# microsoft/ISLE

Measured on AMD Instinct MI355X. Metric: docs/sec end-to-end ISLETrain (SVD+k-means), k=1000; top-k σ rel-err, higher is better.
Workload: dtype f32

## Files before the change

isle_amd/csrc/api.cpp:

```cpp
#include <algorithm>
#include <chrono>
#include <cmath>
#include <cstdarg>
#include <cstdlib>
#include <cstring>
#include <numeric>
#include <thread>

#include <dlfcn.h>

#include "api_internal.h"

int isle_fail(isle_ctx* c, int code, const char* fmt, ...) {
  char buf[1024];
  va_list ap;
  va_start(ap, fmt);
  vsnprintf(buf, sizeof buf, fmt, ap);
  va_end(ap);
  if (c) c->err = buf;
  return code;
}

const IsleKnobInfo isle_knob_table[KN_COUNT] = {
    {"ISLE_GRAM_LDS", "form", "0: Gram apply and k-wide products by the row-gather kernels (any CSC matrix) instead of the LDS-banded form (row-constant B)"},
// ... 6 lines not shown
    {"ISLE_GL_PANEL", "tuning", "8 | 10: columns per pass of the k-wide / thin products (default 10, 8 at 8 items per lane in pass 1)"},
    {"ISLE_GL_WIDE_GROUPED", "tuning", "0: every panel pass of the projection writes its 40 bytes straight into the documents' rows of P (default on a large shard: the panels' rows go whole and in position order into a scratch, sixteen at a time, and a second kernel assembles 640-byte pieces of the document-major rows and the rows' squared norms)"},
    {"ISLE_WIDE_GATHER", "form", "k-wide products (projection, first word-space assignment) by the row-gather kernel"},
    {"ISLE_WIDE_LDS", "form", "k-wide products through the LDS-banded pass-1 stream whatever the vocabulary size"},
    {"ISLE_KS_ROWSHARD", "form", "0: every rank orthogonalises the whole Krylov block (default with several ranks: row slices, all-reduced coefficients, all-gathered block)"},
    {"ISLE_KS_SYNC", "form", "expand loop without the speculative pipeline (one host synchronisation per step)"},
    {"ISLE_KS_ORTHO_PASSES", "form", "3: the reference's three Gram-Schmidt passes per Krylov step instead of two"},
    {"ISLE_UPDATE_MFMA", "form", "0: the orthogonalisation's update F -= V H by FMA chains with the coefficients read from LDS (update_k) instead of on the matrix cores (same sums in another order)"},
    {"ISLE_EVD_JACOBI", "form", "small symmetric EVD by block Jacobi instead of tridiagonalisation"},
    {"ISLE_TD_CHAIN", "form", "tridiagonalisation as a launch chain instead of the persistent kernel"},
    {"ISLE_TD_BAR", "tuning", "flat | hier: the persistent tridiagonalisation crosses its grid barriers on one counter (gb_barrier) or through the hierarchical barrier (gbh_barrier) instead of the sharded counters polled together (gbs_barrier, gridbar.h; round 6: 36.4 / 37.0 / 40.7 ms per EVD at n = 2000 sharded / hier / flat); same bits"},
    {"ISLE_TD_BACK", "form", "seq: the eigenvectors' back-transformation applies the reflectors one by one (td_back_k) instead of by blocks of four in compact WY form"},
    {"ISLE_EVD_SPLIT", "form", "1: with several ranks rank r computes the eigenvectors [r kc, (r + 1) kc) of the small EVD and the columns are all-gathered (same bits on every rank; default since round 6: every rank computes all of them — the stage's kernels are chains of n steps whatever the number of vectors, the split saves no time)"},
    {"ISLE_KMPP_HOST_DICE", "form", "k-means++ dice scaled and searched through the host round trip (the multi-rank form) on one rank too"},
    {"ISLE_KMPP_SPARSE", "form", "0 / 1: k-means++ rounds on the projection / through thin products of B (default: by cost)"},
    {"ISLE_KMPP_TRACK", "form", "0: Lloyd in span(U) always starts with a full assignment pass (default at k > 224 on a large shard: it starts from the nearest seeds and tile minima the k-means++ rounds kept)"},
    {"ISLE_NO_HAMERLY", "form", "both Lloyd loops without distance bounds (every document re-examined every iteration)"},
    {"ISLE_KMEANS_BOUNDS", "form", "hamerly | none: bounds of Lloyd on B (default Yinyang group bounds)"},
    {"ISLE_PROJ_BOUNDS", "form", "hamerly: single lower bound in the projected Lloyd loop at k > 224 instead of tile bounds"},
    {"ISLE_PROJ_FULL", "form", "gemm | fused: full passes of the projected Lloyd loop as GEMM + epilogue or as the fused register kernel"},
    {"ISLE_FIRST_ASSIGN", "form", "sparse | projection: first assignment of Lloyd on B through the sparse product or through the projection"},
    {"ISLE_GEMM_BF16X3", "form", "0: the D x k x k dot products of the assignment steps on the f32 matrix cores (gemm_f32.h) instead of the bf16 ones with operands split in three terms (gemm_bf16x3.h)"},
    {"ISLE_GEMM_EPILOGUE", "form", "0: the D x k x k products of the assignment steps are written to memory and read by dots_assign_cm_k / proj_dots_tiles_k instead of the epilogues inside the product (same bits)"},
    {"ISLE_GEMM_TERMS", "form", "3: the assignment products run once with three bf16 terms per operand (default: two terms first, the rows whose arg-min that leaves open again with three; same assignment)"},
    {"ISLE_GEMM_DMA", "form", "0: the two-term pass of the assignment products splits A on the fly and stages it through registers (gemm_bf16x3_k) instead of reading the projection's pre-split copy by LDS-DMA through a ring of stages (gemm_bf16x2_dma_k; same products in the same order: same bits)"},
    {"ISLE_YY_MODE", "form", "doc | docg | group: Yinyang iteration by document (row-major / group-major centres) or ordered by group (default: group at k >= 256)"},
    {"ISLE_YY_FUSED", "form", "0: the by-group Yinyang iteration lowers the bounds (yy_filter_k) and tightens the active documents (yy2_tighten_k) in two launches instead of one (same bits)"},
    {"ISLE_YY_MOVERS", "form", "0: every centre's movement lowers its Yinyang group's bound (default: up to ten centres that moved far beyond the rest are bounded by their exact new distances instead)"},
    {"ISLE_YY_REGROUP", "form", "0: a Yinyang group is eight consecutive centres (default at k >= 256 behind the product's first assignment: the centres in the order of their squared norms, so that the few centres every far-off document is near share groups; same partitions, a third of the (document, group) pairs)"},
    {"ISLE_YY_ORDER", "form", "doc | member: the Yinyang filter visits the documents in their own order or in the member lists' (default: doc for the fused by-group launch, member otherwise; same bits)"},
// ... 635 lines not shown
```

isle_amd/csrc/common.h:

```cpp
#pragma once
#include <hip/hip_runtime.h>
#include <rccl/rccl.h>

#include <atomic>
#include <cstdint>
#include <cstdio>
#include <functional>
#include <string>
#include <thread>
#include <vector>

struct IsleLaunchRefused {
  const char* file = nullptr;
  int line = 0;
  unsigned long long threads = 0;
};
inline IsleLaunchRefused& isle_launch_refused() {
  static thread_local IsleLaunchRefused r;
  return r;
}
inline bool isle_launch_fits(dim3 g, dim3 b, const char* file, int line) {
  const unsigned long long blocks = (unsigned long long)g.x * g.y * g.z, threads = blocks * ((unsigned long long)b.x * b.y * b.z);
  if (threads < (1ull << 32)) return true;
  IsleLaunchRefused& r = isle_launch_refused();
// ... 56 lines not shown
    hipError_t e = hipHostMalloc((void**)&p, n, hipHostMallocDefault);
    if (e == hipSuccess) cap = n;
    return e;
  }
  PinBuf() = default;
  PinBuf(const PinBuf&) = delete;
  PinBuf& operator=(const PinBuf&) = delete;
  ~PinBuf() {
    if (p) (void)hipHostFree(p);
  }
};

enum IsleKnob {
  KN_GRAM_LDS, KN_GL_G1, KN_GL_G2, KN_GL_PLACE, KN_GL_FILL_BUCKETS, KN_GL_ROUNDS, KN_GL_COLUMNS, KN_GL_PANEL, KN_GL_WIDE_GROUPED, KN_WIDE_GATHER, KN_WIDE_LDS,
  KN_KS_ROWSHARD, KN_KS_SYNC, KN_KS_ORTHO_PASSES, KN_UPDATE_MFMA, KN_EVD_JACOBI, KN_TD_CHAIN, KN_TD_BAR, KN_TD_BACK, KN_EVD_SPLIT,
  KN_KMPP_HOST_DICE, KN_KMPP_SPARSE, KN_KMPP_TRACK, KN_NO_HAMERLY, KN_KMEANS_BOUNDS, KN_PROJ_BOUNDS, KN_PROJ_FULL, KN_FIRST_ASSIGN, KN_GEMM_BF16X3, KN_GEMM_EPILOGUE, KN_GEMM_TERMS, KN_GEMM_DMA, KN_YY_MODE, KN_YY_FUSED, KN_YY_MOVERS, KN_YY_REGROUP, KN_YY_ORDER, KN_PT_SORT, KN_PROJ_ACTIVE, KN_PROJ_SUMS, KN_CENTERS_FRESH,
  KN_INFER_CAP_ROWS, KN_CHUNK_COLS, KN_COMM_TIMEOUT, KN_COMM_SELFTEST, KN_FORCE_COMM, KN_TEST_STALL_MS,
  KN_ROCTX, KN_HOST_TRACE, KN_DEBUG_HAMERLY, KN_DEBUG_EVD, KN_GL_VERBOSE, KN_TD_FORCE_BAIL_RANK, KN_GL_TEST_CUS, KN_GL_ABLATE_SKIP,
  KN_COUNT
};
struct IsleKnobInfo {
  const char* name;
  const char* kind;
  const char* what;
};
extern const IsleKnobInfo isle_knob_table[KN_COUNT];

struct GlDesc {
  uint32_t wave0, wstride, nw, b0, b1, slab, pos_base, pad;
};
struct GlSide {
  uint32_t n_out = 0, n_src = 0, NB = 0, nslice = 0, nwv = 0, ndesc = 0;
  int G = 4;
  uint32_t wpg = 16;
  DevBuf<uint32_t> slice_of;
  DevBuf<int64_t> roff;
  DevBuf<uint16_t> cnt;
  DevBuf<uint2> ids;
  DevBuf<GlDesc> desc;
  int64_t total_sr = 0;
};

struct IslePinSmall {
  double kmpp_stage[(128u << 10) / 8];
// ... 215 lines not shown
  DevBuf<float> ptlb;
  DevBuf<uint32_t> pneed;
  DevBuf<uint32_t> pcand;
  DevBuf<int> seg_desc;
  DevBuf<float> seg_part;
  DevBuf<uint32_t> proj_counted;
  DevBuf<uint32_t> proj_nch;
  DevBuf<float> proj_dpart;
  DevBuf<float> Csum_local;
  DevBuf<uint32_t> active;
  DevBuf<unsigned long long> dbg_cnt;
  DevBuf<uint32_t> kmpp_arg;
  DevBuf<float> kmpp_m2a;
  DevBuf<float> kmpp_tmin;
  DevBuf<float> kmpp_best;
  bool kmpp_track = false;
  int kmpp_track_seeds = 0;
  int kmpp_track_k = 0;
  uint64_t P_gen = 0, kmpp_P_gen = 0;
  std::vector<float> kmpp_C_host;
  DevBuf<float> yy_cg;
  DevBuf<uint32_t> yy_map;
  DevBuf<float> yy_cns;
  DevBuf<float> yy_liftC;
  DevBuf<uint32_t> yy_own, yy_res;
  DevBuf<unsigned long long> yy_need;
  DevBuf<uint32_t> yy_cnt, yy_off;
  DevBuf<uint8_t> yy_pgrp;
  DevBuf<float> centers_old;
  DevBuf<float> Pa, pna, Cold;
// ... 119 lines not shown
int k_ham_delta(isle_ctx* c, float* delta_dev , int k, HamTop* top_dev);
int k_hamerly_filter(isle_ctx* c, const uint32_t* order, const uint32_t* assign, float* ub, float* lb, const float* delta_dev, const HamTop* top_dev,
                     uint32_t* active, uint32_t* nactive, int fam = ISLE_T_SPARSE_ASSIGN);
int k_csc_validate(isle_ctx* c, unsigned long long* err_host2);
int k_doc_norms(isle_ctx* c, float* dn);
int k_centers_from_rows(isle_ctx* c, const uint32_t* assign, int k, int ldk, float* Crm, bool first_of_run = true);
int k_pt_filter(isle_ctx* c, const uint32_t* order, const uint32_t* assign, float* ub, float* tlb, int T, int TL, const float* delta_dev,
                const float* tmove_dev, uint32_t* need, uint32_t* active, uint32_t* nactive, const YyMovers& mv, const float* mdots, const float* cn, const float* pn);
int k_pt_tighten(isle_ctx* c, const float* P, const float* pn, int ldk, const float* C, const float* cn, const uint32_t* assign, const uint32_t* cand,
                 const uint32_t* ncand, float* ub, const float* tlb, int T, int TL, uint32_t* need, uint32_t* active, uint32_t* nactive);
int k_gl_detect(isle_ctx* c);
int k_centers_counts(isle_ctx* c, const uint32_t* assign, int k, int ldk, float* Crm, bool fresh);
int k_gl_build(isle_ctx* c);
int k_gl_wide(isle_ctx* c, const float* Mrm, int k, int ld, float* Out, float* norms = nullptr ,
              void* A2pos = nullptr , bool* a2_done = nullptr);
int k_gl_thin(isle_ctx* c, const float* Wcm, int nc, int ld, float* Out, bool by_position = false);
int k_gl_apply_cm(isle_ctx* c, const float* Xcm, int b, int BP, float* Zcm);
int k_gl_panel_width(const isle_ctx* c);

int k_th_stats(isle_ctx* c, uint64_t* tokens_nz_dev);
int k_th_round_hist(isle_ctx* c, float avg, uint32_t maxv);
int k_th_zetas(isle_ctx* c, uint32_t maxv, uint64_t count_gr, uint64_t count_eq);
int k_th_count(isle_ctx* c, bool with_weights);
int k_th_drop(isle_ctx* c, const uint8_t* drop_dev);
int k_th_scans(isle_ctx* c);
int k_th_emit(isle_ctx* c, uint64_t doc_base);

int k_sort_pairs_u64(isle_ctx* c, uint64_t* key_a, uint32_t* val_a, uint64_t* key_b, uint32_t* val_b, uint64_t n, int key_bits, bool* in_a);
int k_ingest_tdf(isle_ctx* c, const unsigned char* text_dev, uint64_t n, uint64_t V, uint64_t D, uint64_t* entries_read, uint64_t* err_out);
int k_feed_chunk(isle_ctx* c, const uint32_t* docs, const uint32_t* words, const uint32_t* counts, uint64_t n, uint64_t* bad);
int k_feed_finalize(isle_ctx* c);
// ... 108 lines not shown
```

isle_amd/csrc/gram_lds.hip:

```cpp
#include <algorithm>
#include <cstdio>
#include <cstdlib>
#include <vector>

#include "common.h"
#include "scan.h"

namespace {

constexpr int GL_WAVES = 16;
constexpr int GL_THREADS = GL_WAVES * 64;
constexpr int GL_GMAX = 8;
#ifndef GL_RB_V
#define GL_RB_V 4078
#endif
#ifndef GL_APPLY_WAVES_V
#define GL_APPLY_WAVES_V 16
#endif
constexpr uint32_t GL_RB = GL_RB_V;
constexpr uint32_t GL_APPLY_WAVES = GL_APPLY_WAVES_V;
constexpr uint32_t GL_NZ = 16;
constexpr uint32_t GL_PS = GL_RB + GL_NZ;
constexpr uint32_t GL_PSB = GL_PS * 16;
__host__ __device__ constexpr uint32_t gl_img_bytes(int LPE, bool half) { return GL_RB * (16u * (uint32_t)(half ? LPE - 1 : LPE) + (half ? 8u : 0u)); }
// ... 671 lines not shown
#define gl_ld_ids(p) gl_ld_ids_nt(p)
#else
#define gl_ld_ids(p) (*(p))
#endif

#ifndef GL_STAMPS
#define GL_STAMPS 0
#endif
#if GL_STAMPS
__device__ unsigned long long gl_stamp_acc[8];
#define GL_STAMP(var) const unsigned long long var = __builtin_amdgcn_s_memtime()
#else
#define GL_STAMP(var)
#endif

template <int LPE, bool HALF, int G>
__global__ __launch_bounds__(GL_THREADS) void gl_apply_k(const float4* __restrict__ In, uint32_t n_src, const uint2* __restrict__ ids,
                                                          const int64_t* __restrict__ roff, const uint16_t* __restrict__ cnt,
                                                          const uint32_t* __restrict__ slice_of, const GlDesc* __restrict__ desc, uint32_t NB,
                                                          float4* __restrict__ Out, size_t slab_stride, uint32_t n_out,
                                                          const uint32_t* __restrict__ rowmap ,
                                                          uint32_t out_ld4 ,
                                                          uint32_t out_n2 ) {
  extern __shared__ float4 xs[];
  constexpr int NF = HALF ? LPE - 1 : LPE;
  constexpr int NFA = NF > 0 ? NF : 1;
  constexpr uint32_t IMG = gl_img_bytes(LPE, HALF);
  constexpr int NPIECE = NF * 64 + (HALF ? 32 : 0);
  constexpr int GL_INFLIGHT = G * (4 * NF + (HALF ? 2 : 0)) <= 56 ? 4 : 2;
  const GlDesc ds = desc[blockIdx.x];
  const int lane = threadIdx.x & 63;
  const int w = __builtin_amdgcn_readfirstlane((int)(threadIdx.x >> 6));
  const int nwaves = (int)(blockDim.x >> 6);
  const bool wvalid = (uint32_t)w < ds.nw;
  const size_t wv = wvalid ? (size_t)ds.wave0 + (size_t)w * ds.wstride : (size_t)ds.wave0;
  constexpr uint32_t P0 = HALF ? GL_PS * 8u : 0u;
  uint32_t p0s = P0;
  asm volatile("" : "+s"(p0s));
// ... 108 lines not shown
    atomicAdd(&gl_stamp_acc[2], st_b2);
    atomicAdd(&gl_stamp_acc[3], st_walk);
    atomicAdd(&gl_stamp_acc[4], st_sr);
    atomicAdd(&gl_stamp_acc[5], 1ull);
    atomicAdd(&gl_stamp_acc[6], (unsigned long long)(ds.b1 - ds.b0));
  }
#endif
  if (!wvalid) return;
  if ((GL_ABLATE & 64) && (q2.x ^ q3.y) == 0x12345u) acc[0][0].x += 1.f;
  float4* out = Out + (size_t)ds.slab * slab_stride;
#pragma unroll
  for (int g = 0; g < G; ++g) {
    const uint32_t sl = slice_of[wv * G + g];
    const uint64_t pos = (uint64_t)sl * 64 + lane;
    if (sl != GL_NONE && pos < n_out) {
      if (out_n2 == GL_OUT_PLANAR) {
        const uint32_t ob = (uint32_t)pos / GL_RB, orow = (uint32_t)pos - ob * GL_RB;
        char* o = reinterpret_cast<char*>(Out) + (size_t)ob * IMG;
#pragma unroll
        for (int l = 0; l < NF; ++l) *reinterpret_cast<float4*>(o + (size_t)l * GL_RB * 16u + (size_t)orow * 16u) = acc[g][l];
        if (HALF) *reinterpret_cast<float2*>(o + (size_t)NF * GL_RB * 16u + (size_t)orow * 8u) = acch[g];
        continue;
      }
      const size_t row = rowmap ? (size_t)rowmap[pos] : (size_t)(pos - ds.pos_base);
      if (out_n2) {
        float2* o2 = reinterpret_cast<float2*>(out) + row * (size_t)out_ld4 * 2;
#pragma unroll
        for (int l = 0; l < NF; ++l) {
          if (2u * l < out_n2) o2[2 * l] = make_float2(acc[g][l].x, acc[g][l].y);
          if (2u * l + 1 < out_n2) o2[2 * l + 1] = make_float2(acc[g][l].z, acc[g][l].w);
// ... 254 lines not shown
    const bool place = !c->knob_zero(KN_GL_PLACE);
    for (size_t sid0 = 0; sid0 < nsl; sid0 += (size_t)8 << 22) {
      const dim3 grid((unsigned)cdiv((long)std::min<size_t>(nsl - sid0, (size_t)8 << 22), 8));
      if (place) {
        hipLaunchKernelGGL((gl_place_k<4, 0>), grid, dim3(512), 0, c->stream, s.NB, s.G, sid0, nsl, s.cnt.p, s.roff.p, s.ids.p);
        hipLaunchKernelGGL((gl_place_k<GL_PLACE_MAXN, 4>), grid, dim3(512), 0, c->stream, s.NB, s.G, sid0, nsl, s.cnt.p, s.roff.p, s.ids.p);
      }
      hipLaunchKernelGGL(gl_scale_ids_k, grid, dim3(512), 0, c->stream, s.G, sid0, nsl, place ? (uint32_t)GL_PLACE_MAXN : 0u, s.cnt.p, s.roff.p, s.ids.p);
      HIPCHK(c, hipGetLastError());
    }
  }
  HIPCHK(c, hipMemsetD16Async((hipDeviceptr_t)(ids16 + n16_body), (unsigned short)(GL_RB * 8), n16_all - n16_body, c->stream));
  return 0;
}

template <int LPE, bool HALF, int G>
int launch_apply_g(isle_ctx* c, const GlSide& s, const float4* In, float4* Out, size_t slab_stride, const uint32_t* rowmap, uint32_t out_ld4,
                   uint32_t out_n2) {
  constexpr uint32_t lds = (uint32_t)(HALF ? LPE - 1 : LPE) * GL_PSB + (HALF ? GL_PS * 8u : 0u);
  ISLECHK(isle_max_lds(c, (const void*)gl_apply_k<LPE, HALF, G>, (int)lds));
  hipLaunchKernelGGL((gl_apply_k<LPE, HALF, G>), dim3(s.ndesc), dim3(64 * s.wpg), lds, c->stream, In, s.n_src, s.ids.p, s.roff.p, s.cnt.p,
                     s.slice_of.p, s.desc.p, s.NB, Out, slab_stride, s.n_out, rowmap, out_ld4 ? out_ld4 : (uint32_t)LPE, out_n2);
  HIPCHK(c, hipGetLastError());
  return 0;
}
template <int LPE, bool HALF>
int launch_apply(isle_ctx* c, const GlSide& s, const float4* In, float4* Out, size_t slab_stride, const uint32_t* rowmap = nullptr,
                 uint32_t out_ld4 = 0, uint32_t out_n2 = 0) {
  switch (s.G) {
    case 4: return launch_apply_g<LPE, HALF, 4>(c, s, In, Out, slab_stride, rowmap, out_ld4, out_n2);
    case 5: return launch_apply_g<LPE, HALF, 5>(c, s, In, Out, slab_stride, rowmap, out_ld4, out_n2);
    case 6: return launch_apply_g<LPE, HALF, 6>(c, s, In, Out, slab_stride, rowmap, out_ld4, out_n2);
    case 7: return launch_apply_g<LPE, HALF, 7>(c, s, In, Out, slab_stride, rowmap, out_ld4, out_n2);
    case 8: return launch_apply_g<LPE, HALF, 8>(c, s, In, Out, slab_stride, rowmap, out_ld4, out_n2);
  }
  return isle_fail(c, ISLE_E_ARG, "LDS Gram apply: %d items per lane", s.G);
}
int launch_apply_any(isle_ctx* c, int LPE, bool half, const GlSide& s, const float4* In, float4* Out, size_t slab_stride, uint32_t out_n2) {
  if (LPE == 1) return half ? launch_apply<1, true>(c, s, In, Out, slab_stride, nullptr, 0, out_n2) : launch_apply<1, false>(c, s, In, Out, slab_stride, nullptr, 0, out_n2);
  if (LPE == 2) return half ? launch_apply<2, true>(c, s, In, Out, slab_stride, nullptr, 0, out_n2) : launch_apply<2, false>(c, s, In, Out, slab_stride, nullptr, 0, out_n2);
  if (LPE == 3 && half) return launch_apply<3, true>(c, s, In, Out, slab_stride, nullptr, 0, out_n2);
  return isle_fail(c, ISLE_E_ARG, "LDS Gram apply: a panel of %d columns", 4 * LPE);
}
// ... 401 lines not shown
  HIPCHK(c, hipGetLastError());
  return 0;
}

static int gl_panel_width(const isle_ctx* c) {
  const char* e = c->knob(KN_GL_PANEL);
  if (e && atoi(e) == 10) return 10;
  if (e && atoi(e) == 8) return 8;
  return c->gl1.G <= 7 ? 10 : 8;
}

static inline int gl_panel_store_cols(int j0, int ncol, int k, int ld) { return j0 + ncol >= k ? ld - j0 : ncol; }
static inline int gl_panel_cols(int PW, int j0, int k, int ld) { return k - j0 <= PW && ld - j0 > 10 ? 8 : std::min(PW, k - j0); }

static int gl_panel_pass(isle_ctx* c, int wcols, int j0, int ld, float* Out, float* scratch = nullptr ,
                         bool by_position = false ) {
  const int LPE = (wcols + 3) / 4;
  const bool half = wcols <= 4 * LPE - 2;
  const float4* in = (const float4*)c->gl_Xs.p;
  if (scratch) {
    float4* so = (float4*)scratch;
    if (LPE == 1) return half ? launch_apply<1, true>(c, c->gl1, in, so, 0, nullptr, 3, 0) : launch_apply<1, false>(c, c->gl1, in, so, 0, nullptr, 3, 0);
    if (LPE == 2) return half ? launch_apply<2, true>(c, c->gl1, in, so, 0, nullptr, 3, 0) : launch_apply<2, false>(c, c->gl1, in, so, 0, nullptr, 3, 0);
    if (LPE == 3 && half) return launch_apply<3, true>(c, c->gl1, in, so, 0, nullptr, 3, 0);
    return isle_fail(c, ISLE_E_ARG, "LDS products: a panel of %d stored columns", wcols);
  }
  const uint32_t ld4 = (uint32_t)(ld / 4);
  float4* out = (float4*)(Out + j0);
  const uint32_t n2 = (j0 % 4) || half ? (uint32_t)((wcols + 1) / 2) : 0u;
  const uint32_t* rowmap = by_position ? nullptr : c->dperm.p;
  if (LPE == 1) return half ? launch_apply<1, true>(c, c->gl1, in, out, 0, rowmap, ld4, n2) : launch_apply<1, false>(c, c->gl1, in, out, 0, rowmap, ld4, n2);
  if (LPE == 2) return half ? launch_apply<2, true>(c, c->gl1, in, out, 0, rowmap, ld4, n2) : launch_apply<2, false>(c, c->gl1, in, out, 0, rowmap, ld4, n2);
  if (LPE == 3 && half) return launch_apply<3, true>(c, c->gl1, in, out, 0, rowmap, ld4, n2);
  return isle_fail(c, ISLE_E_ARG, "LDS products: a panel of %d stored columns", wcols);
}

int k_gl_panel_width(const isle_ctx* c) { return gl_panel_width(c); }

int k_gl_thin(isle_ctx* c, const float* Wcm, int nc, int ld, float* Out, bool by_position) {
  ISLECHK(k_band_build(c));
  if (c->gl_mode != 1) return isle_fail(c, ISLE_E_ARG, "k_gl_thin needs the LDS-banded form");
  if (ld % 4 || nc > ld) return isle_fail(c, ISLE_E_ARG, "k_gl_thin: bad leading dimension");
  const uint32_t V = (uint32_t)c->V;
  HIPCHK(c, c->gl_Xs.reserve(gl_packed_floats(V, 3, true)));
  const int PW = gl_panel_width(c);
  for (int j0 = 0, ncol; j0 < nc; j0 += ncol) {
    ncol = gl_panel_cols(PW, j0, nc, ld);
    const int wcols = gl_panel_store_cols(j0, ncol, nc, ld);
    const int LPE = (wcols + 3) / 4;
    const bool half = wcols <= 4 * LPE - 2;
    const size_t n4 = (size_t)V * LPE;
    hipLaunchKernelGGL(gl_pack_scale_k, dim3(cdiv((long)n4, 256)), dim3(256), 0, c->stream, Wcm + (size_t)j0 * V, (size_t)V, ncol, LPE, (int)half,
                       c->rowval.p, (char*)c->gl_Xs.p);
    HIPCHK(c, hipGetLastError());
    ISLECHK(gl_panel_pass(c, wcols, j0, ld, Out, nullptr, by_position));
  }
  return 0;
}

constexpr int GL_WG_PANELS = 16;
struct GlWidePanels {
  int n;
  int j0[GL_WG_PANELS];
  int w[GL_WG_PANELS];
  int ncols;
};
__global__ __launch_bounds__(256) void gl_wide_assemble_k(const float* __restrict__ scratch, size_t slab , uint32_t D,
                                                           const uint32_t* __restrict__ rowmap, GlWidePanels g, int jg0, int ld,
                                                           float* __restrict__ Out, float* __restrict__ normpart ,
                                                           uint4* __restrict__ A2 ,
// ... 149 lines not shown
```

isle_amd/csrc/kmeans.hip:

```cpp
#include <algorithm>
#include <cstdlib>
#include <vector>

#include <cstring>

#include "common.h"
#include "hamerly.h"
#include "scan.h"

typedef float floatx16 __attribute__((ext_vector_type(16)));
constexpr int CS_ITEMS = 16;
enum { PR_ARGMIN = 0, PR_MINDIST = 1, PR_TILES = 2 };
template <int MODE>
static int launch_proj_reg(isle_ctx* c, uint64_t D, int k, int ldk, const float* C, const float* cn, const float* pn, uint32_t* assign,
                           float* min_dist, bool* done, const float* Pt = nullptr, const uint32_t* map = nullptr, float* ub = nullptr,
                           float* lb = nullptr, const uint32_t* need = nullptr, int TL = 0);

template <int NIT>
__global__ __launch_bounds__(256) void kmpp_update_k(const float* __restrict__ P, const float* __restrict__ pn, uint32_t D, int ldk,
                                                      const float* __restrict__ newC, const float* __restrict__ cn, int nc,
                                                      float* __restrict__ min_dist) {
  const int lane = threadIdx.x & 63;
  const uint32_t d = blockIdx.x * 4 + (threadIdx.x >> 6);
  if (d >= D) return;
// ... 204 lines not shown
    }
    hamerly_store_bounds(b, m2a[d], nd + tcn[Ta], &uu, &ll);
    rows_s[threadIdx.x][Ta] = ll;
    hamerly_store_bounds(b, b, nd + tcn[32], &uu, &ll);
    ub[d] = uu;
    assign[d] = a;
  }
  __syncthreads();
  const uint32_t nd_blk = min(256u, D - d0);
  for (uint32_t i = threadIdx.x; i < nd_blk * (uint32_t)TL; i += 256) {
    const uint32_t j = i / (uint32_t)TL, t = i - j * (uint32_t)TL;
    if ((int)t < T) tlb[(size_t)d0 * TL + i] = rows_s[j][t];
  }
}

static void launch_min_dots(isle_ctx* c, bool track, int ld, const float* pn, const float* cn, int ncj, uint64_t D, float* min_dist, uint32_t s0) {
  const dim3 g(cdiv(D, 256)), b(256);
#define MD(N)                                                                                                                                     \
  if (track)                                                                                                                                      \
    hipLaunchKernelGGL(kmpp_min_dots_track_k<N>, g, b, 0, c->stream, c->dotsT.p, pn, cn, ncj, (uint32_t)D, min_dist, c->kmpp_arg.p, c->kmpp_m2a.p, \
                       c->kmpp_tmin.p, s0, c->dpos.p);                                                                                            \
  else                                                                                                                                            \
    hipLaunchKernelGGL(kmpp_min_dots_k<N>, g, b, 0, c->stream, c->dotsT.p, pn, cn, ncj, (uint32_t)D, min_dist, c->dpos.p)
  switch (ld / 4) {
    case 1: MD(1); break;
    case 2: MD(2); break;
    case 3: MD(3); break;
    case 4: MD(4); break;
    case 5: MD(5); break;
    case 6: MD(6); break;
// ... 4 lines not shown
}
int k_kmpp_update(isle_ctx* c, const float* P, const float* pn, uint64_t D, int k, int ldk, const float* newC, int nc,
                  float* min_dist, int s_old, bool track) {
  TimeScope ts(c, ISLE_T_KMPP);
  if (D == 0 || nc == 0) return 0;
  if (s_old == 0) c->kmpp_track = false;
  HIPCHK(c, c->cnorm.reserve((size_t)std::max(k, nc)));
  ISLECHK(k_rownorms(c, newC, nc, k, ldk, c->cnorm.p));
  {
    const char* e = c->knob(KN_KMPP_SPARSE);
    const int PW = k_gl_panel_width(c);
    const int passes = (nc + PW - 1) / PW;
    const bool can = c->gl_mode == 1 && c->band_ready && c->U_k == k;
    bool sparse = can && 15.4 * (double)c->nnz * passes < 4.0 * (double)ldk * (double)D * (nc <= 16 ? 1.0 : 2.3);
    if (e) sparse = atoi(e) != 0 && can;
    if (sparse) {
      for (int j0 = 0; j0 < nc; j0 += 32) {
        const int ncj = std::min(32, nc - j0);
        const int ld = (ncj + 3) & ~3;
        HIPCHK(c, c->Tmp.reserve((size_t)c->V * 32));
        HIPCHK(c, c->dotsT.reserve((size_t)D * 32));
        ISLECHK(k_gemm_nn(c, c->Ucm.p, c->V, k, newC + (size_t)j0 * ldk, ldk, ncj, c->Tmp.p, ISLE_T_KMPP));
        ISLECHK(k_gl_thin(c, c->Tmp.p, ncj, ld, c->dotsT.p, true));
        if (track) {
          const int T = (k + 31) / 32;
          if (s_old == 0 && j0 == 0) {
            HIPCHK(c, c->kmpp_arg.reserve(D));
            HIPCHK(c, c->kmpp_m2a.reserve(D));
            HIPCHK(c, c->kmpp_tmin.reserve((size_t)D * T));
            ISLECHK(k_fill_f32(c, c->kmpp_tmin.p, (size_t)D * T, 3.402823466e+38f));
            ISLECHK(k_fill_f32(c, c->kmpp_m2a.p, D, 3.402823466e+38f));
            HIPCHK(c, hipMemsetAsync(c->kmpp_arg.p, 0, D * sizeof(uint32_t), c->stream));
            c->kmpp_track = true;
          }
          if (c->kmpp_track) launch_min_dots(c, true, ld, pn, c->cnorm.p + j0, ncj, D, min_dist, (uint32_t)(s_old + j0));
          else launch_min_dots(c, false, ld, pn, c->cnorm.p + j0, ncj, D, min_dist, 0u);
        } else {
          launch_min_dots(c, false, ld, pn, c->cnorm.p + j0, ncj, D, min_dist, 0u);
        }
        HIPCHK(c, hipGetLastError());
      }
      if (track && c->kmpp_track) c->kmpp_track_seeds = s_old + nc;
      return 0;
    }
  }
  c->kmpp_track = false;
  if (nc <= 16 && (c->Pt_ready || c->Pt2_ready) && (size_t)k * ((nc + 3) / 4) * sizeof(float4) <= 64 * 1024) {
    ISLECHK(k_ensure_pt(c));
    const int nq = (nc + 3) / 4;
    const dim3 g(cdiv(D, 256)), b(256);
    const size_t lds = (size_t)k * nq * sizeof(float4);
#define LP(N) hipLaunchKernelGGL(kmpp_min_pt_k<N>, g, b, lds, c->stream, c->Pt.p, pn, (uint32_t)D, k, ldk, newC, c->cnorm.p, nc, min_dist)
    if (nq == 1) LP(1);
    else if (nq == 2) LP(2);
    else if (nq == 3) LP(3);
    else LP(4);
#undef LP
    HIPCHK(c, hipGetLastError());
    return 0;
  }
  if (nc <= 32) {
// ... 601 lines not shown
    float uu, ll;
    hamerly_store_bounds(m1, m1, nd + tc, &uu, &ll);
    lb[(size_t)d * TL + T] = ll;
  }
  assign[d] = bidx;
  float uu, ll, l2;
  hamerly_store_bounds(best, second, nd + btc, &uu, &l2);
  hamerly_store_bounds(best, best, nd + cmax, &uu, &ll);
  ub[d] = uu;
  lb[(size_t)d * TL + btile] = l2;
}

int k_kmpp_to_tiles(isle_ctx* c, uint64_t D, int k, const float* pn, const float* cn, const float* best, uint32_t* assign, float* ub, int TL) {
  TimeScope ts(c, ISLE_T_LLOYD_PROJ);
  if (D == 0) return 0;
  hipLaunchKernelGGL(kmpp_to_tiles_k, dim3(cdiv(D, 256)), dim3(256), 0, c->stream, (uint32_t)D, k, pn, cn, best, c->kmpp_arg.p, c->kmpp_m2a.p, c->kmpp_tmin.p, assign,
                     ub, c->ptlb.p, TL);
  HIPCHK(c, hipGetLastError());
  return 0;
}

bool k_proj_full_by_gemm(isle_ctx* c, uint64_t D, int k) {
  const char* pf = c->knob(KN_PROJ_FULL);
  return (c->Pt_ready || c->Pt2_ready) && D > 0 && k >= 64 && (k_gemm_assign_fused_ok(c, D, k, k) || isle_scratch_ok(c, c->dotsT.cap, (double)D * k * sizeof(float))) &&
         ((2.0 * (double)D * k * k >= 2e10 && !(pf && !strcmp(pf, "fused"))) || (pf && !strcmp(pf, "gemm")));
}
int k_proj_assign_tiles(isle_ctx* c, const float* P, const float* pn, uint64_t D, int k, int ldk, const float* C, const float* cn, uint32_t* assign,
                        float* ub, float* tlb, int TL, const uint32_t* active, uint32_t n, const uint32_t* need, float* Pa, float* pna) {
  TimeScope ts(c, ISLE_T_LLOYD_PROJ);
  bool done = false;
// ... 519 lines not shown
```

Baseline: 4.767 million.

## Fold k-means++ distance updates into the thin product's last panel epilogue

On a single rank, the k-means++ sparse rounds now fold the min-distance and tile-tracking updates into the epilogue of the LDS-banded thin product's last panel, replacing the separate min_dots kernel. The state is kept by document position (pnp, bestp, tmin by position) so the epilogue can update it without scattering, and a new position-indexed kernel converts it into tile bounds for Lloyd. This removes a launch and a re-read of the stored dots per 32-seed block. In exchange it adds a noinline fold function in the apply kernel that rereads earlier panels' dots, which may raise register pressure or serialise work per lane, plus extra gather and position buffers.

Measured after the change: 4.761 million. Within noise of the previous version (-0.1%).

```diff
diff --git a/isle_amd/csrc/api.cpp b/isle_amd/csrc/api.cpp
--- a/isle_amd/csrc/api.cpp
+++ b/isle_amd/csrc/api.cpp
@@ -44,6 +44,7 @@
     {"ISLE_EVD_SPLIT", "form", "1: with several ranks rank r computes the eigenvectors [r kc, (r + 1) kc) of the small EVD and the columns are all-gathered (same bits on every rank; default since round 6: every rank computes all of them — the stage's kernels are chains of n steps whatever the number of vectors, the split saves no time)"},
     {"ISLE_KMPP_HOST_DICE", "form", "k-means++ dice scaled and searched through the host round trip (the multi-rank form) on one rank too"},
     {"ISLE_KMPP_SPARSE", "form", "0 / 1: k-means++ rounds on the projection / through thin products of B (default: by cost)"},
+    {"ISLE_KMPP_FUSED", "form", "0: k-means++ rounds through thin products fold the distances in a kernel of their own, every panel stored (default on one rank: in the epilogue of the round's last panel, the state kept by position; same bits)"},
     {"ISLE_KMPP_TRACK", "form", "0: Lloyd in span(U) always starts with a full assignment pass (default at k > 224 on a large shard: it starts from the nearest seeds and tile minima the k-means++ rounds kept)"},
     {"ISLE_NO_HAMERLY", "form", "both Lloyd loops without distance bounds (every document re-examined every iteration)"},
     {"ISLE_KMEANS_BOUNDS", "form", "hamerly | none: bounds of Lloyd on B (default Yinyang group bounds)"},
diff --git a/isle_amd/csrc/common.h b/isle_amd/csrc/common.h
--- a/isle_amd/csrc/common.h
+++ b/isle_amd/csrc/common.h
@@ -94,7 +94,7 @@
 enum IsleKnob {
   KN_GRAM_LDS, KN_GL_G1, KN_GL_G2, KN_GL_PLACE, KN_GL_FILL_BUCKETS, KN_GL_ROUNDS, KN_GL_COLUMNS, KN_GL_PANEL, KN_GL_WIDE_GROUPED, KN_WIDE_GATHER, KN_WIDE_LDS,
   KN_KS_ROWSHARD, KN_KS_SYNC, KN_KS_ORTHO_PASSES, KN_UPDATE_MFMA, KN_EVD_JACOBI, KN_TD_CHAIN, KN_TD_BAR, KN_TD_BACK, KN_EVD_SPLIT,
-  KN_KMPP_HOST_DICE, KN_KMPP_SPARSE, KN_KMPP_TRACK, KN_NO_HAMERLY, KN_KMEANS_BOUNDS, KN_PROJ_BOUNDS, KN_PROJ_FULL, KN_FIRST_ASSIGN, KN_GEMM_BF16X3, KN_GEMM_EPILOGUE, KN_GEMM_TERMS, KN_GEMM_DMA, KN_YY_MODE, KN_YY_FUSED, KN_YY_MOVERS, KN_YY_REGROUP, KN_YY_ORDER, KN_PT_SORT, KN_PROJ_ACTIVE, KN_PROJ_SUMS, KN_CENTERS_FRESH,
+  KN_KMPP_HOST_DICE, KN_KMPP_SPARSE, KN_KMPP_FUSED, KN_KMPP_TRACK, KN_NO_HAMERLY, KN_KMEANS_BOUNDS, KN_PROJ_BOUNDS, KN_PROJ_FULL, KN_FIRST_ASSIGN, KN_GEMM_BF16X3, KN_GEMM_EPILOGUE, KN_GEMM_TERMS, KN_GEMM_DMA, KN_YY_MODE, KN_YY_FUSED, KN_YY_MOVERS, KN_YY_REGROUP, KN_YY_ORDER, KN_PT_SORT, KN_PROJ_ACTIVE, KN_PROJ_SUMS, KN_CENTERS_FRESH,
   KN_INFER_CAP_ROWS, KN_CHUNK_COLS, KN_COMM_TIMEOUT, KN_COMM_SELFTEST, KN_FORCE_COMM, KN_TEST_STALL_MS,
   KN_ROCTX, KN_HOST_TRACE, KN_DEBUG_HAMERLY, KN_DEBUG_EVD, KN_GL_VERBOSE, KN_TD_FORCE_BAIL_RANK, KN_GL_TEST_CUS, KN_GL_ABLATE_SKIP,
   KN_COUNT
@@ -108,6 +108,20 @@
 
 struct GlDesc {
   uint32_t wave0, wstride, nw, b0, b1, slab, pos_base, pad;
+};
+struct GlKmppEpi {
+  const float* cn;
+  const float* pn;
+  float* best;
+  uint32_t* arg;
+  float* m2a;
+  float* tmin;
+  float* md_doc;
+  const uint32_t* dperm;
+  const float* dots;
+  uint32_t ld, j0, nc;
+  uint32_t s_old;
+  uint32_t D, track;
 };
 struct GlSide {
   uint32_t n_out = 0, n_src = 0, NB = 0, nslice = 0, nwv = 0, ndesc = 0;
@@ -353,6 +367,9 @@
   DevBuf<float> kmpp_m2a;
   DevBuf<float> kmpp_tmin;
   DevBuf<float> kmpp_best;
+  DevBuf<float> kmpp_pnp, kmpp_bestp;
+  bool kmpp_pos = false;
+  const float* kmpp_bestp_src = nullptr;
   bool kmpp_track = false;
   int kmpp_track_seeds = 0;
   int kmpp_track_k = 0;
@@ -502,7 +519,7 @@
 int k_gl_build(isle_ctx* c);
 int k_gl_wide(isle_ctx* c, const float* Mrm, int k, int ld, float* Out, float* norms = nullptr ,
               void* A2pos = nullptr , bool* a2_done = nullptr);
-int k_gl_thin(isle_ctx* c, const float* Wcm, int nc, int ld, float* Out, bool by_position = false);
+int k_gl_thin(isle_ctx* c, const float* Wcm, int nc, int ld, float* Out, bool by_position = false, const GlKmppEpi* epi = nullptr );
 int k_gl_apply_cm(isle_ctx* c, const float* Xcm, int b, int BP, float* Zcm);
 int k_gl_panel_width(const isle_ctx* c);
 
diff --git a/isle_amd/csrc/gram_lds.hip b/isle_amd/csrc/gram_lds.hip
--- a/isle_amd/csrc/gram_lds.hip
+++ b/isle_amd/csrc/gram_lds.hip
@@ -709,14 +709,92 @@
 #define GL_STAMP(var)
 #endif
 
-template <int LPE, bool HALF, int G>
+struct GlNoEpi {};
+template <bool EPI>
+struct GlEpiArg {
+  typedef GlNoEpi type;
+};
+template <>
+struct GlEpiArg<true> {
+  typedef GlKmppEpi type;
+};
+__device__ __noinline__ void gl_kmpp_fold(const GlKmppEpi& e, size_t row, float4 a0, float4 a1, float2 ah, int nx ) {
+  float xs[10] = {a0.x, a0.y, a0.z, a0.w, a1.x, a1.y, a1.z, a1.w, 0.f, 0.f};
+  if (nx == 2) {
+    xs[0] = ah.x;
+    xs[1] = ah.y;
+  } else if (nx == 6) {
+    xs[4] = ah.x;
+    xs[5] = ah.y;
+  } else if (nx == 10) {
+    xs[8] = ah.x;
+    xs[9] = ah.y;
+  }
+  const float nd = e.pn[row];
+  float m = e.best[row];
+  const float2* prev = reinterpret_cast<const float2*>(e.dots + row * (size_t)e.ld);
+  const uint32_t nq = e.j0 >> 1;
+  if (!e.track) {
+#pragma nounroll
+    for (uint32_t q = 0; q < nq; ++q) {
+      const float2 v = prev[q];
+      m = fminf(m, fmaxf((-2.0f * v.x + e.cn[2 * q]) + nd, 0.0f));
+      m = fminf(m, fmaxf((-2.0f * v.y + e.cn[2 * q + 1]) + nd, 0.0f));
+    }
+#pragma unroll
+    for (int t = 0; t < 10; ++t)
+      if (t < nx && e.j0 + (uint32_t)t < e.nc) m = fminf(m, fmaxf((-2.0f * xs[t] + e.cn[e.j0 + t]) + nd, 0.0f));
+    e.best[row] = m;
+    e.md_doc[e.dperm[row]] = m;
+    return;
+  }
+  float m2 = e.m2a[row];
+  uint32_t ar = e.arg[row];
+  float* tm_col = e.tmin + row;
+  uint32_t curT = e.s_old >> 5;
+  float tm = tm_col[(size_t)curT * e.D];
+  auto fold = [&](uint32_t j, float dot) {
+    const uint32_t sj = e.s_old + j, T = sj >> 5;
+    if (T != curT) {
+      tm_col[(size_t)curT * e.D] = tm;
+      curT = T;
+      tm = tm_col[(size_t)T * e.D];
+    }
+    const float x = fmaxf((-2.0f * dot + e.cn[j]) + nd, 0.0f);
+    if (x < m) {
+      m2 = (T == (ar >> 5) && m < 3.0e38f) ? m : tm;
+      m = x;
+      ar = sj;
+    } else if (T == (ar >> 5)) {
+      m2 = fminf(m2, x);
+    }
+    tm = fminf(tm, x);
+  };
+#pragma nounroll
+  for (uint32_t q = 0; q < nq; ++q) {
+    const float2 v = prev[q];
+    fold(2 * q, v.x);
+    fold(2 * q + 1, v.y);
+  }
+#pragma unroll
+  for (int t = 0; t < 10; ++t)
+    if (t < nx && e.j0 + (uint32_t)t < e.nc) fold(e.j0 + (uint32_t)t, xs[t]);
+  tm_col[(size_t)curT * e.D] = tm;
+  e.best[row] = m;
+  e.arg[row] = ar;
+  e.m2a[row] = m2;
+  e.md_doc[e.dperm[row]] = m;
+}
+
+template <int LPE, bool HALF, int G, bool EPI = false>
 __global__ __launch_bounds__(GL_THREADS) void gl_apply_k(const float4* __restrict__ In, uint32_t n_src, const uint2* __restrict__ ids,
                                                           const int64_t* __restrict__ roff, const uint16_t* __restrict__ cnt,
                                                           const uint32_t* __restrict__ slice_of, const GlDesc* __restrict__ desc, uint32_t NB,
                                                           float4* __restrict__ Out, size_t slab_stride, uint32_t n_out,
                                                           const uint32_t* __restrict__ rowmap ,
                                                           uint32_t out_ld4 ,
-                                                          uint32_t out_n2 ) {
+                                                          uint32_t out_n2 ,
+                                                          typename GlEpiArg<EPI>::type epi ) {
   extern __shared__ float4 xs[];
   constexpr int NF = HALF ? LPE - 1 : LPE;
   constexpr int NFA = NF > 0 ? NF : 1;
@@ -855,6 +933,10 @@
     const uint32_t sl = slice_of[wv * G + g];
     const uint64_t pos = (uint64_t)sl * 64 + lane;
     if (sl != GL_NONE && pos < n_out) {
+      if constexpr (EPI) {
+        gl_kmpp_fold(epi, (size_t)(pos - ds.pos_base), acc[g][0], NF > 1 ? acc[g][NFA - 1] : make_float4(0.f, 0.f, 0.f, 0.f), acch[g], 4 * NF + (HALF ? 2 : 0));
+        continue;
+      }
       if (out_n2 == GL_OUT_PLANAR) {
         const uint32_t ob = (uint32_t)pos / GL_RB, orow = (uint32_t)pos - ob * GL_RB;
         char* o = reinterpret_cast<char*>(Out) + (size_t)ob * IMG;
@@ -1139,19 +1221,31 @@
   return 0;
 }
 
-template <int LPE, bool HALF, int G>
+template <int LPE, bool HALF, int G, bool EPI = false>
 int launch_apply_g(isle_ctx* c, const GlSide& s, const float4* In, float4* Out, size_t slab_stride, const uint32_t* rowmap, uint32_t out_ld4,
-                   uint32_t out_n2) {
+                   uint32_t out_n2, const GlKmppEpi* epi = nullptr) {
   constexpr uint32_t lds = (uint32_t)(HALF ? LPE - 1 : LPE) * GL_PSB + (HALF ? GL_PS * 8u : 0u);
-  ISLECHK(isle_max_lds(c, (const void*)gl_apply_k<LPE, HALF, G>, (int)lds));
-  hipLaunchKernelGGL((gl_apply_k<LPE, HALF, G>), dim3(s.ndesc), dim3(64 * s.wpg), lds, c->stream, In, s.n_src, s.ids.p, s.roff.p, s.cnt.p,
-                     s.slice_of.p, s.desc.p, s.NB, Out, slab_stride, s.n_out, rowmap, out_ld4 ? out_ld4 : (uint32_t)LPE, out_n2);
+  typename GlEpiArg<EPI>::type ea{};
+  if constexpr (EPI) ea = *epi;
+  ISLECHK(isle_max_lds(c, (const void*)gl_apply_k<LPE, HALF, G, EPI>, (int)lds));
+  hipLaunchKernelGGL((gl_apply_k<LPE, HALF, G, EPI>), dim3(s.ndesc), dim3(64 * s.wpg), lds, c->stream, In, s.n_src, s.ids.p, s.roff.p, s.cnt.p,
+                     s.slice_of.p, s.desc.p, s.NB, Out, slab_stride, s.n_out, rowmap, out_ld4 ? out_ld4 : (uint32_t)LPE, out_n2, ea);
   HIPCHK(c, hipGetLastError());
   return 0;
 }
 template <int LPE, bool HALF>
 int launch_apply(isle_ctx* c, const GlSide& s, const float4* In, float4* Out, size_t slab_stride, const uint32_t* rowmap = nullptr,
-                 uint32_t out_ld4 = 0, uint32_t out_n2 = 0) {
+                 uint32_t out_ld4 = 0, uint32_t out_n2 = 0, const GlKmppEpi* epi = nullptr) {
+  if (epi) {
+    switch (s.G) {
+      case 4: return launch_apply_g<LPE, HALF, 4, true>(c, s, In, Out, slab_stride, nullptr, out_ld4, out_n2, epi);
+      case 5: return launch_apply_g<LPE, HALF, 5, true>(c, s, In, Out, slab_stride, nullptr, out_ld4, out_n2, epi);
+      case 6: return launch_apply_g<LPE, HALF, 6, true>(c, s, In, Out, slab_stride, nullptr, out_ld4, out_n2, epi);
+      case 7: return launch_apply_g<LPE, HALF, 7, true>(c, s, In, Out, slab_stride, nullptr, out_ld4, out_n2, epi);
+      case 8: return launch_apply_g<LPE, HALF, 8, true>(c, s, In, Out, slab_stride, nullptr, out_ld4, out_n2, epi);
+    }
+    return isle_fail(c, ISLE_E_ARG, "LDS Gram apply: %d items per lane", s.G);
+  }
   switch (s.G) {
     case 4: return launch_apply_g<LPE, HALF, 4>(c, s, In, Out, slab_stride, rowmap, out_ld4, out_n2);
     case 5: return launch_apply_g<LPE, HALF, 5>(c, s, In, Out, slab_stride, rowmap, out_ld4, out_n2);
@@ -1583,7 +1677,8 @@
 static inline int gl_panel_cols(int PW, int j0, int k, int ld) { return k - j0 <= PW && ld - j0 > 10 ? 8 : std::min(PW, k - j0); }
 
 static int gl_panel_pass(isle_ctx* c, int wcols, int j0, int ld, float* Out, float* scratch = nullptr ,
-                         bool by_position = false ) {
+                         bool by_position = false ,
+                         const GlKmppEpi* epi = nullptr ) {
   const int LPE = (wcols + 3) / 4;
   const bool half = wcols <= 4 * LPE - 2;
   const float4* in = (const float4*)c->gl_Xs.p;
@@ -1598,15 +1693,16 @@
   float4* out = (float4*)(Out + j0);
   const uint32_t n2 = (j0 % 4) || half ? (uint32_t)((wcols + 1) / 2) : 0u;
   const uint32_t* rowmap = by_position ? nullptr : c->dperm.p;
-  if (LPE == 1) return half ? launch_apply<1, true>(c, c->gl1, in, out, 0, rowmap, ld4, n2) : launch_apply<1, false>(c, c->gl1, in, out, 0, rowmap, ld4, n2);
-  if (LPE == 2) return half ? launch_apply<2, true>(c, c->gl1, in, out, 0, rowmap, ld4, n2) : launch_apply<2, false>(c, c->gl1, in, out, 0, rowmap, ld4, n2);
-  if (LPE == 3 && half) return launch_apply<3, true>(c, c->gl1, in, out, 0, rowmap, ld4, n2);
+  if (epi && !by_position) return isle_fail(c, ISLE_E_ARG, "LDS products: the k-means++ epilogue needs rows by position");
+  if (LPE == 1) return half ? launch_apply<1, true>(c, c->gl1, in, out, 0, rowmap, ld4, n2, epi) : launch_apply<1, false>(c, c->gl1, in, out, 0, rowmap, ld4, n2, epi);
+  if (LPE == 2) return half ? launch_apply<2, true>(c, c->gl1, in, out, 0, rowmap, ld4, n2, epi) : launch_apply<2, false>(c, c->gl1, in, out, 0, rowmap, ld4, n2, epi);
+  if (LPE == 3 && half) return launch_apply<3, true>(c, c->gl1, in, out, 0, rowmap, ld4, n2, epi);
   return isle_fail(c, ISLE_E_ARG, "LDS products: a panel of %d stored columns", wcols);
 }
 
 int k_gl_panel_width(const isle_ctx* c) { return gl_panel_width(c); }
 
-int k_gl_thin(isle_ctx* c, const float* Wcm, int nc, int ld, float* Out, bool by_position) {
+int k_gl_thin(isle_ctx* c, const float* Wcm, int nc, int ld, float* Out, bool by_position, const GlKmppEpi* epi) {
   ISLECHK(k_band_build(c));
   if (c->gl_mode != 1) return isle_fail(c, ISLE_E_ARG, "k_gl_thin needs the LDS-banded form");
   if (ld % 4 || nc > ld) return isle_fail(c, ISLE_E_ARG, "k_gl_thin: bad leading dimension");
@@ -1622,7 +1718,17 @@
     hipLaunchKernelGGL(gl_pack_scale_k, dim3(cdiv((long)n4, 256)), dim3(256), 0, c->stream, Wcm + (size_t)j0 * V, (size_t)V, ncol, LPE, (int)half,
                        c->rowval.p, (char*)c->gl_Xs.p);
     HIPCHK(c, hipGetLastError());
-    ISLECHK(gl_panel_pass(c, wcols, j0, ld, Out, nullptr, by_position));
+    if (epi && j0 + ncol >= nc) {
+      if (c->gl1.n_out != (uint32_t)c->D || (j0 & 1)) return isle_fail(c, ISLE_E_ARG, "k_gl_thin: the k-means++ epilogue does not fit this stream");
+      GlKmppEpi e = *epi;
+      e.dots = Out;
+      e.ld = (uint32_t)ld;
+      e.j0 = (uint32_t)j0;
+      e.nc = (uint32_t)nc;
+      ISLECHK(gl_panel_pass(c, wcols, j0, ld, Out, nullptr, by_position, &e));
+    } else {
+      ISLECHK(gl_panel_pass(c, wcols, j0, ld, Out, nullptr, by_position));
+    }
   }
   return 0;
 }
diff --git a/isle_amd/csrc/kmeans.hip b/isle_amd/csrc/kmeans.hip
--- a/isle_amd/csrc/kmeans.hip
+++ b/isle_amd/csrc/kmeans.hip
@@ -242,6 +242,61 @@
   }
 }
 
+__global__ __launch_bounds__(256) void kmpp_to_tiles_pos_k(uint32_t D, int k, const float* __restrict__ pnp, const float* __restrict__ cn,
+                                                            const float* __restrict__ bestp, const uint32_t* __restrict__ argp,
+                                                            const float* __restrict__ m2ap, const float* __restrict__ tminp,
+                                                            const uint32_t* __restrict__ dperm, uint32_t* __restrict__ assign,
+                                                            float* __restrict__ ub, float* __restrict__ tlb, int TL) {
+  __shared__ float tcn[33];
+  const int T = (k + 31) / 32;
+  if (threadIdx.x < 33) {
+    float m = 0.f;
+    if ((int)threadIdx.x < T)
+      for (int j = 32 * threadIdx.x; j < min(k, 32 * (int)threadIdx.x + 32); ++j) m = fmaxf(m, cn[j]);
+    tcn[threadIdx.x] = m;
+  }
+  __syncthreads();
+  if (threadIdx.x == 0) {
+    float m = 0.f;
+    for (int t = 0; t < T; ++t) m = fmaxf(m, tcn[t]);
+    tcn[32] = m;
+  }
+  __syncthreads();
+  __shared__ float rows_s[256][33];
+  __shared__ uint32_t doc_s[256];
+  const uint32_t p0 = blockIdx.x * 256, p = p0 + threadIdx.x;
+  if (p < D) {
+    const float nd = pnp[p], b = bestp[p];
+    const uint32_t a = argp[p], Ta = a >> 5, d = dperm[p];
+    float uu, ll;
+    for (int t = 0; t < T; ++t) {
+      const float m1 = tminp[(size_t)t * D + p];
+      hamerly_store_bounds(m1, m1, nd + tcn[t], &uu, &ll);
+      rows_s[threadIdx.x][t] = ll;
+    }
+    hamerly_store_bounds(b, m2ap[p], nd + tcn[Ta], &uu, &ll);
+    rows_s[threadIdx.x][Ta] = ll;
+    hamerly_store_bounds(b, b, nd + tcn[32], &uu, &ll);
+    ub[d] = uu;
+    assign[d] = a;
+    doc_s[threadIdx.x] = d;
+  }
+  __syncthreads();
+  const uint32_t np_blk = min(256u, D - p0);
+  for (uint32_t i = threadIdx.x; i < np_blk * (uint32_t)TL; i += 256) {
+    const uint32_t j = i / (uint32_t)TL, t = i - j * (uint32_t)TL;
+    if ((int)t < T) tlb[(size_t)doc_s[j] * TL + t] = rows_s[j][t];
+  }
+}
+__global__ __launch_bounds__(256) void kmpp_gather_pos_k(const float* __restrict__ pn, const float* __restrict__ md, const uint32_t* __restrict__ dperm,
+                                                          uint32_t D, float* __restrict__ pnp, float* __restrict__ bestp) {
+  const uint32_t p = blockIdx.x * 256 + threadIdx.x;
+  if (p >= D) return;
+  const uint32_t d = dperm[p];
+  pnp[p] = pn[d];
+  bestp[p] = md[d];
+}
+
 static void launch_min_dots(isle_ctx* c, bool track, int ld, const float* pn, const float* cn, int ncj, uint64_t D, float* min_dist, uint32_t s0) {
   const dim3 g(cdiv(D, 256)), b(256);
 #define MD(N)                                                                                                                                     \
@@ -276,17 +331,40 @@
     const bool can = c->gl_mode == 1 && c->band_ready && c->U_k == k;
     bool sparse = can && 15.4 * (double)c->nnz * passes < 4.0 * (double)ldk * (double)D * (nc <= 16 ? 1.0 : 2.3);
     if (e) sparse = atoi(e) != 0 && can;
+    const bool fused = sparse && !c->knob_zero(KN_KMPP_FUSED) && !c->multi() && c->dperm.p != nullptr;
+    if (!fused) c->kmpp_bestp_src = nullptr;
     if (sparse) {
+      HIPCHK(c, c->Tmp.reserve((size_t)c->V * 32));
+      HIPCHK(c, c->dotsT.reserve((size_t)D * 32));
+      if (c->kmpp_track && c->kmpp_pos != fused) c->kmpp_track = false;
+      if (fused && (s_old <= 0 || c->kmpp_bestp_src != min_dist)) {
+        HIPCHK(c, c->kmpp_pnp.reserve(D));
+        HIPCHK(c, c->kmpp_bestp.reserve(D));
+        hipLaunchKernelGGL(kmpp_gather_pos_k, dim3(cdiv(D, 256)), dim3(256), 0, c->stream, pn, min_dist, c->dperm.p, (uint32_t)D, c->kmpp_pnp.p, c->kmpp_bestp.p);
+        HIPCHK(c, hipGetLastError());
+        c->kmpp_bestp_src = min_dist;
+      }
+      if (fused && c->knob_on(KN_DEBUG_HAMERLY)) fprintf(stderr, "[k-means++] %d new seeds folded in the thin product's epilogue%s\n", nc, track ? "" : " (no tracking)");
       for (int j0 = 0; j0 < nc; j0 += 32) {
         const int ncj = std::min(32, nc - j0);
         const int ld = (ncj + 3) & ~3;
-        HIPCHK(c, c->Tmp.reserve((size_t)c->V * 32));
-        HIPCHK(c, c->dotsT.reserve((size_t)D * 32));
         ISLECHK(k_gemm_nn(c, c->Ucm.p, c->V, k, newC + (size_t)j0 * ldk, ldk, ncj, c->Tmp.p, ISLE_T_KMPP));
-        ISLECHK(k_gl_thin(c, c->Tmp.p, ncj, ld, c->dotsT.p, true));
+        GlKmppEpi epi{};
+        if (fused) {
+          epi.cn = c->cnorm.p + j0;
+          epi.pn = c->kmpp_pnp.p;
+          epi.best = c->kmpp_bestp.p;
+          epi.md_doc = min_dist;
+          epi.dperm = c->dperm.p;
+          epi.s_old = (uint32_t)(s_old + j0);
+          epi.D = (uint32_t)D;
+        } else {
+          ISLECHK(k_gl_thin(c, c->Tmp.p, ncj, ld, c->dotsT.p, true));
+        }
         if (track) {
           const int T = (k + 31) / 32;
           if (s_old == 0 && j0 == 0) {
+            c->kmpp_pos = fused;
             HIPCHK(c, c->kmpp_arg.reserve(D));
             HIPCHK(c, c->kmpp_m2a.reserve(D));
             HIPCHK(c, c->kmpp_tmin.reserve((size_t)D * T));
@@ -295,11 +373,22 @@
             HIPCHK(c, hipMemsetAsync(c->kmpp_arg.p, 0, D * sizeof(uint32_t), c->stream));
             c->kmpp_track = true;
           }
-          if (c->kmpp_track) launch_min_dots(c, true, ld, pn, c->cnorm.p + j0, ncj, D, min_dist, (uint32_t)(s_old + j0));
-          else launch_min_dots(c, false, ld, pn, c->cnorm.p + j0, ncj, D, min_dist, 0u);
-        } else {
+          if (fused) {
+            if (c->kmpp_track) {
+              epi.arg = c->kmpp_arg.p;
+              epi.m2a = c->kmpp_m2a.p;
+              epi.tmin = c->kmpp_tmin.p;
+              epi.track = 1u;
+            }
+          } else if (c->kmpp_track) {
+            launch_min_dots(c, true, ld, pn, c->cnorm.p + j0, ncj, D, min_dist, (uint32_t)(s_old + j0));
+          } else {
+            launch_min_dots(c, false, ld, pn, c->cnorm.p + j0, ncj, D, min_dist, 0u);
+          }
+        } else if (!fused) {
           launch_min_dots(c, false, ld, pn, c->cnorm.p + j0, ncj, D, min_dist, 0u);
         }
+        if (fused) ISLECHK(k_gl_thin(c, c->Tmp.p, ncj, ld, c->dotsT.p, true, &epi));
         HIPCHK(c, hipGetLastError());
       }
       if (track && c->kmpp_track) c->kmpp_track_seeds = s_old + nc;
@@ -307,6 +396,7 @@
     }
   }
   c->kmpp_track = false;
+  c->kmpp_bestp_src = nullptr;
   if (nc <= 16 && (c->Pt_ready || c->Pt2_ready) && (size_t)k * ((nc + 3) / 4) * sizeof(float4) <= 64 * 1024) {
     ISLECHK(k_ensure_pt(c));
     const int nq = (nc + 3) / 4;
@@ -938,6 +1028,13 @@
 int k_kmpp_to_tiles(isle_ctx* c, uint64_t D, int k, const float* pn, const float* cn, const float* best, uint32_t* assign, float* ub, int TL) {
   TimeScope ts(c, ISLE_T_LLOYD_PROJ);
   if (D == 0) return 0;
+  if (c->kmpp_pos) {
+    if (c->kmpp_bestp_src != best) return isle_fail(c, ISLE_E_ARG, "k_kmpp_to_tiles: the state by position does not belong to these distances");
+    hipLaunchKernelGGL(kmpp_to_tiles_pos_k, dim3(cdiv(D, 256)), dim3(256), 0, c->stream, (uint32_t)D, k, c->kmpp_pnp.p, cn, c->kmpp_bestp.p, c->kmpp_arg.p,
+                       c->kmpp_m2a.p, c->kmpp_tmin.p, c->dperm.p, assign, ub, c->ptlb.p, TL);
+    HIPCHK(c, hipGetLastError());
+    return 0;
+  }
   hipLaunchKernelGGL(kmpp_to_tiles_k, dim3(cdiv(D, 256)), dim3(256), 0, c->stream, (uint32_t)D, k, pn, cn, best, c->kmpp_arg.p, c->kmpp_m2a.p, c->kmpp_tmin.p, assign,
                      ub, c->ptlb.p, TL);
   HIPCHK(c, hipGetLastError());
```
